# sp-uhh/disentangled-vae

Hardware: AMD Instinct MI355X
Metric: spectrogram frames/sec (train step), M2 VAE 513-bin (higher is better)
Workload: dtype bf16x3; 1 GPU; M2 VAE train step (fwd+ELBO+bwd+Adam), x_dim 513, y_dim 513, z 16, h [128,128], 8192 frames/step/GPU, 16 kHz / 1024-pt STFT power frames; parallelism=dp1, min_hbm_bytes_per_frame=4168

## Files before the change

### disentangled-vae_amd/csrc/rows_common.hpp

```cpp
#pragma once
#include "fused_tiles.hpp"
#include "apply_types.hpp"
#include "../../include/dvae_train.h"

namespace dvae {
namespace fused {

__device__ __forceinline__ void philox_normal4(unsigned long long seed, unsigned long long frame, unsigned long long step, unsigned draw,
                                               float (&out)[4]) {
    unsigned c0 = (unsigned)frame, c1 = (unsigned)(frame >> 32), c2 = (unsigned)step, c3 = ((unsigned)(step >> 32) << 8) | draw;
    unsigned k0 = (unsigned)seed, k1 = (unsigned)(seed >> 32);
#pragma unroll
    for (int r = 0; r < 10; ++r) {
        const unsigned h0 = __umulhi(0xD2511F53u, c0), l0 = 0xD2511F53u * c0;
        const unsigned h1 = __umulhi(0xCD9E8D57u, c2), l1 = 0xCD9E8D57u * c2;
        c0 = h1 ^ c1 ^ k0; c1 = l1; c2 = h0 ^ c3 ^ k1; c3 = l0;
        k0 += 0x9E3779B9u; k1 += 0xBB67AE85u;
    }
    const float u0 = ((float)(c0 >> 8) + 0.5f) * (1.f / 16777216.f), u1 = ((float)(c1 >> 8) + 0.5f) * (1.f / 16777216.f);
    const float u2 = ((float)(c2 >> 8) + 0.5f) * (1.f / 16777216.f), u3 = ((float)(c3 >> 8) + 0.5f) * (1.f / 16777216.f);
    const float ra = sqrtf(-2.f * __logf(u0)), rb = sqrtf(-2.f * __logf(u2));
    float sa, ca, sb, cb;
    __sincosf(6.283185307179586f * u1, &sa, &ca);
    __sincosf(6.283185307179586f * u3, &sb, &cb);
// ... 129 lines not shown
                if (fbase + l31 >= col_limit) f[j] = P::cvt(0.f);
            }
            stash_store16(dbase, (l31 * E + gq * 32 * E) * (int)sizeof(T), f);
        }
    }
}

template <typename P, bool F16 = false, typename RowOf>
__device__ __forceinline__ void load_rows_to_lds(const float* __restrict__ src, int ld, int ncols, int pcols, int64_t b0, int64_t B,
                                                 typename P::T* U, int ldu, int tid, RowOf rowof, float* xf = nullptr,
                                                 float* log2sum = nullptr, float eps = 0.f) {
    const int total = TB * pcols;
    for (int idx = tid; idx < total; idx += 256) {
        const int row = idx / pcols, col = idx - row * pcols;
        float v = 0.f;
        if (col < ncols && b0 + row < B) {
            v = src[rowof(row) * ld + col];
            if (log2sum && col < XD - 1) *log2sum += __builtin_amdgcn_logf(v + eps);
        }
        if constexpr (F16 && P::NP == 2) {
            const float vs = v * X16::XS;
            const typename P::T vh = X16::hi<typename P::T>(vs);
            U[row * ldu + col] = vh;
            U[Pl<P>::lds + row * ldu + col] = X16::hi<typename P::T>(vs - X16::val(vh));
        } else {
            const typename P::T vh = P::cvt(v);
            U[row * ldu + col] = vh;
            if constexpr (P::NP == 2) U[Pl<P>::lds + row * ldu + col] = P::cvt(v - (float)vh);
        }
        if (xf && col < ncols) xf[row * ncols + col] = v;
    }
}

constexpr int NQ513 = 17;
struct __attribute__((packed, aligned(4))) F4U { f32x4 v; };
#ifndef R2_IN_NT
#define R2_IN_NT 0
#endif
typedef f32x4 f32x4_a4 __attribute__((aligned(4)));
__device__ __forceinline__ f32x4 ld_in4(const float* p) {
#if R2_IN_NT >= 1
    return __builtin_nontemporal_load(reinterpret_cast<const f32x4_a4*>(p));
#else
    return reinterpret_cast<const F4U*>(p)->v;
#endif
}
__device__ __forceinline__ f32x4 ld_in4_again(const float* p) {
#if R2_IN_NT >= 2
    return __builtin_nontemporal_load(reinterpret_cast<const f32x4_a4*>(p));
#else
    return reinterpret_cast<const F4U*>(p)->v;
#endif
}
template <int I0, int I1, typename RowOf>
__device__ __forceinline__ void tile513_issue_part(const float* __restrict__ base, RowOf rowof, f32x4 (&v)[NQ513], int tid) {
#pragma unroll
    for (int i = I0; i < I1; ++i) {
        const int c = tid + 256 * i;
        v[i] = ld_in4(base + rowof(c >> 7) * XD + 4 * (c & 127));
    }
}
template <typename RowOf>
__device__ __forceinline__ void tile513_issue_last(const float* __restrict__ base, RowOf rowof, f32x4 (&v)[NQ513], int tid) {
    v[16][0] = base[rowof(tid & 31) * XD + XD - 1];
}
template <typename RowOf>
__device__ __forceinline__ void tile513_issue(const float* __restrict__ base, RowOf rowof, f32x4 (&v)[NQ513], int tid) {
    tile513_issue_part<0, 16>(base, rowof, v, tid);
    tile513_issue_last(base, rowof, v, tid);
    __builtin_amdgcn_sched_barrier(0);
}
template <typename P, int I0, int I1, bool F16 = false>
__device__ __forceinline__ void tile513_commit_part(const f32x4 (&v)[NQ513], typename P::T* U, int ldu, int tid, float* xf, unsigned long long& lo_bits) {
    typedef typename P::Pack4 Pack4;
#pragma unroll
    for (int i = I0; i < I1; ++i) {
        const int c = tid + 256 * i;
        const int row = c >> 7, col = 4 * (c & 127);
        if (xf) {
            float* d = xf + row * XD + col;
            d[0] = v[i][0]; d[1] = v[i][1]; d[2] = v[i][2]; d[3] = v[i][3];
        }
        if constexpr (F16 && P::NP == 2) {
            Pack4 pk, pl;
#pragma unroll
            for (int j = 0; j < 4; ++j) {
                const float vs = v[i][j] * X16::XS;
                pk[j] = X16::hi<typename P::T>(vs);
                pl[j] = X16::hi<typename P::T>(vs - X16::val(pk[j]));
            }
            *reinterpret_cast<Pack4*>(U + row * ldu + col) = pk;
            *reinterpret_cast<Pack4*>(U + Pl<P>::lds + row * ldu + col) = pl;
            continue;
        }
        Pack4 pk;
        pk[0] = P::cvt(v[i][0]); pk[1] = P::cvt(v[i][1]); pk[2] = P::cvt(v[i][2]); pk[3] = P::cvt(v[i][3]);
        *reinterpret_cast<Pack4*>(U + row * ldu + col) = pk;
        if constexpr (P::NP == 2) {
            Pack4 pl;
            pl[0] = P::cvt(v[i][0] - (float)pk[0]); pl[1] = P::cvt(v[i][1] - (float)pk[1]);
            pl[2] = P::cvt(v[i][2] - (float)pk[2]); pl[3] = P::cvt(v[i][3] - (float)pk[3]);
            *reinterpret_cast<Pack4*>(U + Pl<P>::lds + row * ldu + col) = pl;
            lo_bits |= __builtin_bit_cast(unsigned long long, pl) & 0x7fff7fff7fff7fffull;
        }
    }
}
template <typename P, int PCOLS, bool F16 = false>
__device__ __forceinline__ void tile513_commit_last(const f32x4 (&v)[NQ513], typename P::T* U, int ldu, int tid, float* xf, unsigned long long& lo_bits) {
    constexpr int PADC = PCOLS - XD;
    if (tid < TB) {
        if (xf) xf[tid * XD + XD - 1] = v[16][0];
        if constexpr (F16 && P::NP == 2) {
            const float vs = v[16][0] * X16::XS;
            const typename P::T vh = X16::hi<typename P::T>(vs);
            U[tid * ldu + XD - 1] = vh;
            U[Pl<P>::lds + tid * ldu + XD - 1] = X16::hi<typename P::T>(vs - X16::val(vh));
        } else {
        const typename P::T vh = P::cvt(v[16][0]);
        U[tid * ldu + XD - 1] = vh;
        if constexpr (P::NP == 2) {
            const typename P::T vl = P::cvt(v[16][0] - (float)vh);
            U[Pl<P>::lds + tid * ldu + XD - 1] = vl;
            if ((float)vl != 0.f) lo_bits |= 1ull;
        }
        }
    }
    for (int idx = tid; idx < TB * PADC; idx += 256) {
        const int r = idx / PADC, c = XD + idx - r * PADC;
        U[r * ldu + c] = P::cvt(0.f);
        if constexpr (P::NP == 2) U[Pl<P>::lds + r * ldu + c] = P::cvt(0.f);
    }
// ... 98 lines not shown
```

### disentangled-vae_amd/csrc/rows_helper.inc

```
        const int hw = wave_u - ROWS_CHAIN_WAVES, ht = tid - 64 * ROWS_CHAIN_WAVES;
        constexpr bool XFH = P::XF16 && NP == 2;
        constexpr int NBT = Ld<T>::nbias;
        constexpr int NB = (NBT + 255) / 256;
        float bvv[NB];
        auto load_bias = [&]() __attribute__((always_inline)) {
#pragma unroll
            for (int q = 0; q < NB; ++q) {
                int i = ht + 256 * q;
                i = i < NBT ? i : NBT - 1;
                const float* src;
                int k;
                if (i < OB2) { src = g.b1; k = i; }
                else if (i < OBMV) { src = g.b2; k = i - OB2; }
                else if (i < OBMV + ZD) { src = g.bmu; k = i - OBMV; }
                else if (i < OB3) { src = g.blv; k = i - OBMV - ZD; }
                else if (i < OB4) { src = g.b3; k = i - OB3; }
                else if (i < OB5) { src = g.b4; k = i - OB4; }
                else if (i < OB5 + NO) { src = g.b5; k = i - OB5; k = k < XD ? k : XD - 1; }
                else { src = g.w5last; k = i - OB5 - NO; }
                if constexpr (DEFER) bvv[q] = __hip_atomic_load(src + k, __ATOMIC_RELAXED, __HIP_MEMORY_SCOPE_AGENT);
                else bvv[q] = src[k];
            }
        };
        auto store_bias = [&]() __attribute__((always_inline)) {
// ... 5 lines not shown
        };
        if constexpr (!DEFER) load_bias();
        auto fill_rows = [&](int tl_, int half) {
            if (ht < TB) {
                const int64_t bf = (int64_t)tl_ * TB + ht;
                const int64_t br = bf < g.B ? bf : g.B - 1;
                int64_t r = g.rows[br];
                if (r < 0 || r >= g.n_rows) { r = 0; if (g.bad_rows && bf < g.B) atomicAdd(g.bad_rows, 1); }
                rowsrc[half * TB + ht] = r;
            }
        };
        typedef Sched<P, YP, YENC, (OFFL ? P::PDO : P::PD), INFO> SCc;
        typedef HSched<P, YP, YENC, DH, INFO> HS;
        typedef WStream<P, HS, DH> HWS;
        HWS hws;
        if constexpr (HS::any) {
            hws.rs = __builtin_amdgcn_make_buffer_rsrc(const_cast<void*>(g.wcopy), 0, (int)g.wcopy_bytes, 0x00020000);
            hws.voff = lane * 16;
            hws.pl = g.wpl_bytes;
            auto mo = [&](const void* Wp) { return (unsigned)((const char*)Wp - (const char*)g.wcopy); };
            constexpr unsigned FBB = HS::FBB;
            const unsigned tw = (unsigned)hw * FBB;
            hws.sb[H_W1X] = mo(g.W1s) + tw + (unsigned)SCc::NX1 * 4u * FBB;
            hws.sb[H_W3Y] = mo(g.W3s) + tw + (unsigned)(ZD / KS) * 4u * FBB;
            hws.sb[H_W3Z] = mo(g.W3s) + tw;
            hws.sb[H_PAD] = mo(g.W1s);
            if constexpr (INFO) { hws.sb[H_C1] = mo(g.Wc1s) + tw;  hws.sb[H_C2] = mo(g.Wc2s) + tw;  hws.sb[H_C2T] = mo(g.Wc2t) + tw; }
            else { hws.sb[H_C1] = hws.sb[H_C2] = hws.sb[H_C2T] = 0; }
            if constexpr (INFO) hws.fill();
        }
        const T* const Urh = U + l31 * LDU + h * E;
        const T* const Zbrh = Zb + l31 * LDZ + h * E;
        float lsum2 = 0.f;
        f32x4 xv[NQ513], yv[NQ513];
        bool x_in_regs = false;
        bool y_in_regs = false;
        const bool st1 = MODE != 1 && !(g.ablate & 1), st2 = MODE != 1 && !(g.ablate & 2) && (g.stash_inputs & 2), st2x = MODE != 1 && !(g.ablate & 2) && (g.stash_inputs & 1);
        for (int it = 0; it < ntl; ++it) {
            const int tile = tile0 + it * (int)gridDim.x;
            const int64_t b0 = (int64_t)tile * TB;
            const bool full = (b0 + TB) <= g.B;
            const int64_t* const rsrc = rowsrc + (it & 1) * TB;
            auto rowof = [&](int r) -> int64_t {
                if (gather) return rsrc[r];
                const int64_t br = b0 + r;
                return br < g.B ? br : g.B - 1;
            };
            int tl = ht;
            asm volatile("" : "+v"(tl));
            const bool yfast = Y513 && g.fasty && full;
            bool y_early = it > 0 && y_in_regs;
            if (it == 0) {
                if (gather) { fill_rows(tile, 0); wg_barrier(); }
                if (g.fastx && full) {
                    tile513_issue(g.x, rowof, xv, tl);
                    if constexpr (!DEFER) store_bias();
#if R2_EARLY_Y
                    if (YP > 0 && Y513 && g.fasty) {
                        unsigned long long lb = 0ull;
                        static_for<0, 4>([&](auto qc) {
                            constexpr int Q = decltype(qc)::value;
                            tile513_issue_part<4 * Q, 4 * Q + 4>(g.y, rowof, yv, tl);
                            __builtin_amdgcn_sched_barrier(0);
                            tile513_commit_part<P, 4 * Q, 4 * Q + 4, XFH>(xv, U, LDU, tl, nullptr, lb);
                            __builtin_amdgcn_sched_barrier(0);
                        });
                        tile513_issue_last(g.y, rowof, yv, tl);
                        __builtin_amdgcn_sched_barrier(0);
                        tile513_commit_last<P, ROWS_XP, XFH>(xv, U, LDU, tl, nullptr, lb);
                        y_early = true;
                    } else
#endif
                    {
                        tile513_commit<P, ROWS_XP, XFH>(xv, U, LDU, tl);
#pragma unroll
                        for (int i = 0; i < NQ513; ++i) yv[i] = f32x4{0.f, 0.f, 0.f, 0.f};
                    }
                } else {
#pragma unroll
                    for (int i = 0; i < NQ513; ++i) { xv[i] = f32x4{0.f, 0.f, 0.f, 0.f}; yv[i] = f32x4{0.f, 0.f, 0.f, 0.f}; }
                    if constexpr (!DEFER) store_bias();
                    load_rows_to_lds<P, XFH>(g.x, g.ldx, XD, ROWS_XP, b0, g.B, U, LDU, tl, rowof, nullptr, OFFL ? &lsum2 : nullptr, g.elbo_eps);
                }
                if constexpr (INFO) {
                    for (int i = ht; i < 6 * HD + 2; i += 256) {
                        const int q = i / HD, k = i - q * HD;
                        float v;
                        if (q == 0) v = g.bc1[k]; else if (q == 1) v = g.bc2[k]; else if (q == 2) v = g.wc3[k];
                        else if (q == 3) v = g.ba1[k]; else if (q == 4) v = g.ba2[k]; else if (q == 5) v = g.wa3[k];
                        else v = k == 0 ? g.bc3[0] : g.ba3[0];
                        Binfo[i] = v;
                    }
                }
                if (ht == 0) flags[0] = 0;
                if constexpr (DEFER) {
                    wg_barrier();
                    load_bias();
                    store_bias();
                }
                wg_barrier();
                if constexpr (OFFL) { if (g.fastx && full) lsum2 += tile513_log2sum(xv, g.elbo_eps, tl); }
            }
            if constexpr (HS::n(H_W1X) > 0) {
                f32x16 hacc;
                zero_acc<P>(hacc);
                hws.fill();
                gemm_seg<P, HS, DH, H_W1X, HWS, XFH>(hacc, hws, Urh + SCc::NX1 * 2 * E);
#pragma unroll
                for (int r = 0; r < 16; ++r) keep[r * 256 + ht] = XFH ? hacc[r] * X16::ACC : hacc[r];
            }
            float c1r[16], c2r[16], w3c[16];
            float bce_c = 0.f, ylab = 0.f;
            if constexpr (INFO) {
                ylab = g.y[rowof(l31) * g.ldy];
                if (it > 0) hws.fill();
                f32x16 cacc;
                zero_acc<P>(cacc);
                gemm_seg<P, HS, DH, H_C1, HWS, XFH>(cacc, hws, Urh);
                float bvc[16];
                bias16(Binfo + OBC1, 32 * hw, h, bvc);
#pragma unroll
                for (int r = 0; r < 16; ++r) c1r[r] = fmaxf((XFH ? cacc[r] * X16::ACC : cacc[r]) + bvc[r], 0.f);
            }
            f32x16 accy;
            int yplanes = NP;
            int ydirty = 0;
            if constexpr (NP == 2 && YP > 0) { if (g.ylo_skip && st2) ydirty = g.ylo_dirty[tile]; }
            if (YP > 0) {
                if (Y513 && yfast && !y_early) tile513_issue(g.y, rowof, yv, tl);
                R2_HSTAMP(16);
                if (st2x && !XFH) stash_from_lds<P>(U, LDU, ROWS_XP, NO, (T*)g.xT, g.spl, g.Bp, b0, tl);
                R2_HSTAMP(17);
                wg_barrier();
                if constexpr (HS::HELPY && HS::n(H_W1X) == 0) hws.fill();
                R2_HSTAMP(18);
                bool any = false;
                if (Y513 && yfast) tile513_commit<P, ROWS_XP>(yv, U, LDU, tl, nullptr, NP == 2 ? &any : nullptr);
                else load_rows_to_lds<P>(g.y, g.ldy, g.ydim, YP, b0, g.B, U, LDU, tl, rowof);
                R2_HSTAMP(19);
                if constexpr (NP == 2) {
                    if (Y513 && yfast) {
                    } else {
                        constexpr int YPD = YP > 0 ? YP : 1;
                        for (int idx = tl; idx < TB * YP; idx += 256) any |= (float)U[Pl<P>::lds + (idx / YPD) * LDU + idx % YPD] != 0.f;
                    }
                    if (__ballot(any) != 0ull && lane == 0) atomicOr(&flags[0], 1);
                }
                R2_HSTAMP(20);
                if constexpr (INFO) put_lds<P>(c1r, U + IMA, LDU, 32 * hw, l31, h);
                wg_barrier();
                if constexpr (NP == 2) {
                    const bool ylo_t = __builtin_amdgcn_readfirstlane(flags[0]) != 0;
                    if (g.ylo_skip && st2) {
                        ydirty = __builtin_amdgcn_readfirstlane(ydirty);
                        yplanes = (ylo_t || ydirty != 0) ? 2 : 1;
                        if (ht == 0) {
                            if (ylo_t) *g.ylo_epoch = g.launch_id;
                            if ((ylo_t ? 1 : 0) != ydirty) g.ylo_dirty[tile] = ylo_t ? 1 : 0;
                        }
                    }
                }
#if !R2_LATE_Y
                if (st2) stash_from_lds<P>(U, LDU, YP, (YP + 31) / 32 * 32, (T*)g.yT, g.spl, g.Bp, b0, tl, 0, 1 << 30, yplanes);
#endif
                if constexpr (HS::HELPY) {
                    const bool ylo = NP == 2 && __builtin_amdgcn_readfirstlane(flags[0]) != 0;
                    zero_acc<P>(accy);
                    if (!R2_YLOSEG) gemm_seg<P, HS, DH, H_W3Y>(accy, hws, Urh, ylo);
                    else if (ylo) gemm_seg<P, HS, DH, H_W3Y>(accy, hws, Urh, true);
                    else gemm_seg<P, HS, DH, H_W3Y>(accy, hws, Urh, false);
                }
                if constexpr (INFO) {
                    f32x16 a2c;
                    zero_acc<P>(a2c);
                    gemm_seg<P, HS, DH, H_C2>(a2c, hws, Urh + IMA);
                    float bvc[16];
                    bias16(Binfo + OBC2, 32 * hw, h, bvc);
                    bias16(Binfo + OWC3, 32 * hw, h, w3c);
                    float pd = 0.f;
#pragma unroll
                    for (int r = 0; r < 16; ++r) { c2r[r] = fmaxf(a2c[r] + bvc[r], 0.f); pd = fmaf(w3c[r], c2r[r], pd); }
                    put_lds<P>(c2r, U + IMB, LDU, 32 * hw, l31, h);
                    pd += __shfl_xor(pd, 32, 64);
                    if (h == 0) red2[hw * 32 + l31] = pd;
                }
            } else {
                if (st2x && !XFH) stash_from_lds<P>(U, LDU, ROWS_XP, NO, (T*)g.xT, g.spl, g.Bp, b0, tl);
                if constexpr (HS::n(H_W1X) > 0) wg_barrier();
            }
            wg_barrier();
            if constexpr (INFO) {
                const bool live_h = (b0 + l31) < g.B;
                const float logit = red2[l31] + red2[32 + l31] + red2[64 + l31] + red2[96 + l31] + Binfo[OS3];
                const float p = 1.f / (1.f + P::exp_(-logit));
                const float lp = P::log_(p + g.elbo_eps), lq = P::log_(1.f - p + g.elbo_eps);
                bce_c = (live_h && h == 0 && hw == 0) ? -(ylab * lp + (1.f - ylab) * lq) : 0.f;
                const float u = live_h ? -g.invB * (ylab / (p + g.elbo_eps) - (1.f - ylab) / (1.f - p + g.elbo_eps)) : 0.f;
                const float dpre3 = u * p * (1.f - p);
                float dv2[16];
#pragma unroll
                for (int r = 0; r < 16; ++r) dv2[r] = c2r[r] > 0.f ? w3c[r] * dpre3 : 0.f;
                put_lds<P>(dv2, U + IMC, LDU, 32 * hw, l31, h);
                if (st1) {
                    stash_tile<P>(U + IMA, LDU, 32 * hw, (T*)g.c1T + (int64_t)hw * 32 * g.Bp, g.spl, b0, l31, h);
                    stash_tile<P>(U + IMB, LDU, 32 * hw, (T*)g.c2T + (int64_t)hw * 32 * g.Bp, g.spl, b0, l31, h);
                    if (hw == 0 && h == 0) {
                        T* d3 = (T*)g.dc3T + (b0 / KS) * (64 * E) + (l31 / E) * 32 * E + (l31 % E);
                        const T d3h = P::cvt(dpre3 * g.alpha);
                        *d3 = d3h;
                        if constexpr (NP == 2) d3[g.spl] = P::cvt(dpre3 * g.alpha - (float)d3h);
                    }
                }
            }
            if (st1) stash_tile<P>(Ha, LDH, 32 * hw, (T*)g.h1T + (int64_t)hw * 32 * g.Bp, g.spl, b0, l31, h);
#ifndef R2_XSP
#define R2_XSP 1
#endif
            if constexpr (XFH && !INFO && R2_XSP == 0) { if (st2x) xstash_reload<P, 0, 4>(g.x, g.ldx, rowof, b0, g.B, (T*)g.xT, g.spl, g.Bp, tl); }
#if R2_LATE_Y
            if (YP > 0 && st2) stash_from_lds<P>(U, LDU, YP, (YP + 31) / 32 * 32, (T*)g.yT, g.spl, g.Bp, b0, tl, 0, R2_YSPREAD, yplanes);
#endif
            wg_barrier();
            if constexpr (INFO) {
                f32x16 a3c;
                zero_acc<P>(a3c);
                gemm_seg<P, HS, DH, H_C2T>(a3c, hws, Urh + IMC);
                float dv1[16];
#pragma unroll
                for (int r = 0; r < 16; ++r) dv1[r] = c1r[r] > 0.f ? a3c[r] : 0.f;
                put_lds<P>(dv1, U + IMA, LDU, 32 * hw, l31, h);
                if (st1) stash_tile<P>(U + IMC, LDU, 32 * hw, (T*)g.dc2T + (int64_t)hw * 32 * g.Bp, g.spl, b0, l31, h, g.alpha);
            }
            if (st1) stash_tile<P>(Hb, LDH, 32 * hw, (T*)g.h2T + (int64_t)hw * 32 * g.Bp, g.spl, b0, l31, h);
            if constexpr (XFH && !INFO) {
                if (st2x) {
                    if constexpr (R2_XSP == 0) xstash_reload<P, 4, 9>(g.x, g.ldx, rowof, b0, g.B, (T*)g.xT, g.spl, g.Bp, tl);
                    else if constexpr (R2_XSP == 1) xstash_reload<P, 0, 9>(g.x, g.ldx, rowof, b0, g.B, (T*)g.xT, g.spl, g.Bp, tl);
                    else xstash_reload<P, 0, 5>(g.x, g.ldx, rowof, b0, g.B, (T*)g.xT, g.spl, g.Bp, tl);
                }
            }
#if R2_LATE_Y
            if (YP > 0 && st2) stash_from_lds<P>(U, LDU, YP, (YP + 31) / 32 * 32, (T*)g.yT, g.spl, g.Bp, b0, tl, R2_YSPREAD, 1 << 30, yplanes);
#endif
            wg_barrier();
            if constexpr (HS::HELPY) {
                f32x16 az;
                zero_acc<P>(az);
                gemm_seg<P, HS, DH, H_W3Z>(az, hws, Zbrh);
                float hv[16], bv[16];
                bias16(Bias + OB3, 32 * hw, h, bv);
#pragma unroll
                for (int r = 0; r < 16; ++r) hv[r] = P::tanh_(az[r] + accy[r] + bv[r]);
                put_lds<P>(hv, Ha, LDH, 32 * hw, l31, h);
            }
            if (hw == 0 && st1) stash_tile<P>(Zb, LDZ, 0, (T*)g.zT, g.spl, b0, l31, h);
            if constexpr (XFH && !INFO && R2_XSP == 2) { if (st2x) xstash_reload<P, 5, 9>(g.x, g.ldx, rowof, b0, g.B, (T*)g.xT, g.spl, g.Bp, tl); }
            if (ht == 0) flags[0] = 0;
            if constexpr (INFO) {
                if (st1) stash_tile<P>(U + IMA, LDU, 32 * hw, (T*)g.dc1T + (int64_t)hw * 32 * g.Bp, g.spl, b0, l31, h, g.alpha);
                const float sa = g.gamma - g.beta;
                wg_barrier();
                if (st1) stash_tile<P>(Ha, LDH, 32 * hw, (T*)g.a1T + (int64_t)hw * 32 * g.Bp, g.spl, b0, l31, h);
                if constexpr (XFH) { if (st2x) xstash_reload<P, 0, 5>(g.x, g.ldx, rowof, b0, g.B, (T*)g.xT, g.spl, g.Bp, tl); }
                wg_barrier();
                if (st1) {
                    stash_tile<P>(Hb, LDH, 32 * hw, (T*)g.a2T + (int64_t)hw * 32 * g.Bp, g.spl, b0, l31, h);
                    if (hw == 0 && h == 0) {
                        const bool live_h = (b0 + l31) < g.B;
                        const float logit = red2[l31] + red2[32 + l31] + red2[64 + l31] + red2[96 + l31] + Binfo[OS3 + 1];
                        const float p = 1.f / (1.f + P::exp_(-logit));
                        const float u = live_h ? -g.invB * (ylab / (p + g.elbo_eps) - (1.f - ylab) / (1.f - p + g.elbo_eps)) : 0.f;
                        const float dpre3 = u * p * (1.f - p);
                        T* d3 = (T*)g.da3T + (b0 / KS) * (64 * E) + (l31 / E) * 32 * E + (l31 % E);
                        const T d3h = P::cvt(dpre3 * sa);
// ... 137 lines not shown
```

### disentangled-vae_amd/csrc/rows_prologue.inc

```
    typedef typename P::T T;
    typedef typename P::Frag Frag;
    constexpr int E = P::E, KS = P::KSTEP, NP = P::NP;
    constexpr int LDU = Ld<T>::u, LDH = Ld<T>::hh, LDZ = Ld<T>::z;
    constexpr bool Y513 = (YP == ROWS_XP);
#ifndef R2_OFFL
#define R2_OFFL 1
#endif
#ifndef R2_LATE_Y
#define R2_LATE_Y 1
#endif
#ifndef R2_EARLY_Y
#define R2_EARLY_Y 1
#endif
#ifndef R2_DH
#define R2_DH 6
#endif
#ifndef R2_HPRIO
#define R2_HPRIO 0
#endif
#ifndef R2_YSPREAD
#define R2_YSPREAD 8
#endif
#ifndef R2_YLOSEG
#define R2_YLOSEG 0
#endif
#ifndef R2_STAGGER
#define R2_STAGGER 0
#endif
    constexpr bool OFFL = R2_OFFL && MODE == 0 && NP == 2;
    extern __shared__ __attribute__((aligned(16))) char smem[];
    T* const U = reinterpret_cast<T*>(smem);
    T* const Ha = U + TB * LDU;
    T* const Hb = Ha + TB * LDH;
    T* const Zb = Hb + TB * LDH;
    typedef Lds2<P, INFO> LD2;
    float* const Bias = reinterpret_cast<float*>(smem + LD2::o_bias);
    float* const red = reinterpret_cast<float*>(smem + LD2::o_red);
    int* const flags = reinterpret_cast<int*>(smem + LD2::o_flags);
    int64_t* const rowsrc = reinterpret_cast<int64_t*>(smem + LD2::o_rows);
    float* const Binfo = reinterpret_cast<float*>(smem + LD2::o_info);
    float* const red2 = reinterpret_cast<float*>(smem + LD2::o_red2);
    float* const dzs = reinterpret_cast<float*>(smem + LD2::o_dzu);
    constexpr int OBC1 = 0, OBC2 = HD, OWC3 = 2 * HD, OBA1 = 3 * HD, OBA2 = 4 * HD, OWA3 = 5 * HD, OS3 = 6 * HD;
    constexpr int IMA = 32, IMB = 160, IMC = 288;
    float* const keep = reinterpret_cast<float*>(smem + LD2::o_keep);
    float* const keepz = reinterpret_cast<float*>(smem + LD2::o_keepz);
    constexpr int OB1 = 0, OB2 = HD, OBMV = 2 * HD, OB3 = 2 * HD + 32, OB4 = 3 * HD + 32, OB5 = 4 * HD + 32;

    constexpr int DH = R2_DH;
    const int tid = threadIdx.x, lane = tid & 63;
    const int wave_u = __builtin_amdgcn_readfirstlane(tid >> 6);
    const int l31 = lane & 31, h = lane >> 5;
    const bool gather = g.rows != nullptr;
#ifndef R2_XCDMAP
#define R2_XCDMAP 0
#endif
    int tile0 = (int)blockIdx.x;
#if R2_XCDMAP
    if ((gridDim.x & 7) == 0 && (g.ntiles % (int)gridDim.x) == 0) tile0 = (int)(blockIdx.x & 7) * (int)(gridDim.x >> 3) + (int)(blockIdx.x >> 3);
#endif
    const int ntl = (g.ntiles - tile0 + (int)gridDim.x - 1) / (int)gridDim.x;
```

### disentangled-vae_amd/csrc/train_rows2.hip

```cpp
#include <math.h>
#include <stdlib.h>
#include "fused_tiles.hpp"
#include "rows_common.hpp"
#include "wstream.hpp"
#include "apply_common.hpp"
#include "rows_shared.hpp"
#include "../../include/dvae_train.h"

namespace dvae {
namespace fused {

template <typename P, int YP, bool YENC, int MODE, bool INFO = false, bool DEFER = false>
__global__ __launch_bounds__(512) void vae_rows2_kernel(const RowsArgs g) {
    static_assert(!INFO || (MODE == 0 && YP == 16 && !YENC), "M2_info: train step, 1-dim label, encoder on x only");
    static_assert(!DEFER || (MODE == 0 && !INFO && sizeof(typename P::T) == 2), "deferred optimizer step: M1 / M2 train step, bf16 copies");
#define ROWS_XP XP
#define ROWS_PREFETCH 1
#define ROWS_CHAIN_WAVES 4
#include "rows_prologue.inc"
    if (wave_u < 4) {
        const int cw = wave_u, fb = 32 * cw;
        constexpr int D = OFFL ? P::PDO : P::PD;
        typedef Sched<P, YP, YENC, D, INFO> SC;
        typedef HSched<P, YP, YENC, DH, INFO> HS;
#ifndef R2_DEFER_WAUX
#define R2_DEFER_WAUX 0
#endif
        typedef WStream<P, SC, D, DEFER ? R2_DEFER_WAUX : R2_WAUX> WS;
        constexpr unsigned FBB = SC::FBB;
        WS ws;
        ws.rs = __builtin_amdgcn_make_buffer_rsrc(const_cast<void*>(g.wcopy), 0, (int)g.wcopy_bytes, 0x00020000);
        ws.voff = lane * 16;
        ws.pl = g.wpl_bytes;
        {
            auto mo = [&](const void* Wp) { return (unsigned)((const char*)Wp - (const char*)g.wcopy); };
#ifdef R2_SAMEW
            const unsigned tw = 0;
#else
            const unsigned tw = (unsigned)cw * FBB;
#endif
            constexpr unsigned KB1 = (XP / KS) * 4 * FBB, KB3 = (ZD / KS) * 4 * FBB;
            ws.sb[G_W1X] = mo(g.W1s) + tw;  ws.sb[G_W1Y] = mo(g.W1s) + tw + KB1;
            ws.sb[G_W2] = mo(g.W2s) + tw;   ws.sb[G_WMV] = mo(g.Wmvs);
            ws.sb[G_W3Y] = mo(g.W3s) + tw + KB3;  ws.sb[G_W3Z] = mo(g.W3s) + tw;
            ws.sb[G_W4] = mo(g.W4s) + tw;
            ws.sb[G_W5A] = mo(g.W5s) + (unsigned)cw * FBB;        ws.sb[G_W5B] = mo(g.W5s) + (unsigned)(cw + 4) * FBB;
            ws.sb[G_W5C] = mo(g.W5s) + (unsigned)(cw + 8) * FBB;  ws.sb[G_W5D] = mo(g.W5s) + (unsigned)(cw + 12) * FBB;
            ws.sb[G_W5T] = mo(g.W5t) + tw;  ws.sb[G_W4T] = mo(g.W4t) + tw;  ws.sb[G_W3ZT] = mo(g.W3zt);
            ws.sb[G_WMVT] = mo(g.Wmvt) + tw;  ws.sb[G_W2T] = mo(g.W2t) + tw;  ws.sb[G_PAD] = mo(g.W1s);
            if constexpr (INFO) {
                ws.sb[G_A1] = mo(g.Wa1s) + tw;  ws.sb[G_A2] = mo(g.Wa2s) + tw;  ws.sb[G_A2T] = mo(g.Wa2t) + tw;  ws.sb[G_A1T] = mo(g.Wa1t);
            } else { ws.sb[G_A1] = ws.sb[G_A2] = ws.sb[G_A2T] = ws.sb[G_A1T] = 0; }
        }
        if constexpr (DEFER) {
            if (g.defer.have) {
                T* const tile = reinterpret_cast<T*>(keep) + cw * DeferLds<T, NP>::wave_elems;
                if (!(g.defer.diag & 1))
                for (int un = cw * (int)gridDim.x + (int)blockIdx.x; un < 4 * g.defer.ntasks; un += 4 * (int)gridDim.x)
                    defer_unit<T, NP>(g.defer.a, g.defer.tasks[un >> 2], un & 3, tile, lane, g.defer.diag);
                asm volatile("s_waitcnt vmcnt(0)" ::: "memory");
                if (lane == 0)
                    __hip_atomic_fetch_add(g.defer.shard + 32 * (((int)blockIdx.x * 4 + cw) & (DEFER_SHARDS - 1)), 1u, __ATOMIC_RELAXED, __HIP_MEMORY_SCOPE_AGENT);
                if (cw == 0 && !(g.defer.diag & 2)) {
                    const int nw = 4 * (int)gridDim.x, sh = lane & (DEFER_SHARDS - 1);
                    const unsigned want = g.defer.seq_arrive * (unsigned)((nw - sh + DEFER_SHARDS - 1) / DEFER_SHARDS);
                    const unsigned long long deadline = wall_clock64() + g.defer.timeout_ticks;
                    bool ok = true;
                    for (unsigned it_ = 0;; ++it_) {
                        const unsigned have = __hip_atomic_load(g.defer.shard + 32 * sh, __ATOMIC_RELAXED, __HIP_MEMORY_SCOPE_AGENT);
                        if (__ballot((int)(have - want) < 0) == 0ull) break;
                        if ((it_ & 15u) == 0u && wall_clock64() >= deadline) { ok = false; break; }
                        __builtin_amdgcn_s_sleep(1);
                    }
                    if (!ok && lane == 0) __hip_atomic_store(g.defer.err, 1u, __ATOMIC_RELAXED, __HIP_MEMORY_SCOPE_AGENT);
                }
            }
            wg_barrier();
        }
        ws.fill();
        const T* const Ur = U + l31 * LDU + h * E;
        const T* const Har = Ha + l31 * LDH + h * E;
        const T* const Hbr = Hb + l31 * LDH + h * E;
        const T* const Zbr = Zb + l31 * LDZ + h * E;
        const bool w0 = cw == 0;
        constexpr int mode = MODE;
        double tot_rec = 0.0, tot_kl = 0.0, tot_bc = 0.0, tot_ba = 0.0;

        for (int it = 0; it < ntl; ++it) {
            const int tile = tile0 + it * (int)gridDim.x;
            const int64_t b0 = (int64_t)tile * TB;
            const bool live = (b0 + l31) < g.B;
            const int64_t* const rsrc = rowsrc + (it & 1) * TB;
            float rec_lane = 0.f, kl_lane = 0.f;
            R2_STAMP(0);
            if (g.dbg && tid == 0) g.dbg[(size_t)blockIdx.x * 32 + 30] = clock64();
            float ep_r[8];
            if (w0) {
                int64_t br = b0 + l31; br = br < g.B ? br : g.B - 1;
                if (g.eps != nullptr) {
                    const f32x4 e0 = *reinterpret_cast<const f32x4*>(g.eps + br * ZD + 4 * h);
                    const f32x4 e1 = *reinterpret_cast<const f32x4*>(g.eps + br * ZD + 8 + 4 * h);
#pragma unroll
                    for (int jq = 0; jq < 4; ++jq) { ep_r[jq] = live ? e0[jq] : 0.f; ep_r[4 + jq] = live ? e1[jq] : 0.f; }
                } else {
                    frame_noise8(g.rng_seed, (unsigned long long)br, g.rng_step, h, ep_r);
#pragma unroll
                    for (int jq = 0; jq < 8; ++jq) ep_r[jq] = live ? ep_r[jq] : 0.f;
                }
            }
            if (it == 0) {
                if (gather) wg_barrier();
                wg_barrier();
            }
            R2_STAMP(1);
#if R2_STAGGER
            if (it == 0) { for (int q = 0; q < (int)((blockIdx.x >> 3) & 7); ++q) __builtin_amdgcn_s_sleep(R2_STAGGER); }
#endif
            f32x16 acc;
            zero_acc<P>(acc);
            constexpr bool XF = P::XF16 && NP == 2;
            gemm_seg<P, SC, D, G_W1X, WS, XF>(acc, ws, Ur);
            if constexpr (XF) {
#pragma unroll
                for (int r = 0; r < 16; ++r) acc[r] *= X16::ACC;
            }
            R2_STAMP(2);
            bool ylo = false;
            if (YP > 0) {
                wg_barrier();
                wg_barrier();
                ylo = NP == 2 && __builtin_amdgcn_readfirstlane(flags[0]) != 0;
                if (!R2_YLOSEG) gemm_seg<P, SC, D, G_W1Y>(acc, ws, Ur, ylo);
                else if (ylo) gemm_seg<P, SC, D, G_W1Y>(acc, ws, Ur, true);
                else gemm_seg<P, SC, D, G_W1Y>(acc, ws, Ur, false);
            } else if constexpr (HS::n(H_W1X) > 0) wg_barrier();
            if constexpr (HS::n(H_W1X) > 0) {
#pragma unroll
                for (int r = 0; r < 16; ++r) acc[r] += keep[r * 256 + tid];
            }
            float hv[16], bv[16];
            R2_STAMP(3);
            bias16(Bias + OB1, fb, h, bv);
#pragma unroll
            for (int r = 0; r < 16; ++r) { hv[r] = P::tanh_(acc[r] + bv[r]); keep[r * 256 + tid] = hv[r]; }
            put_lds<P>(hv, Ha, LDH, fb, l31, h);
            wg_barrier();
            R2_STAMP(4);
            zero_acc<P>(acc);
            gemm_seg<P, SC, D, G_W2>(acc, ws, Har);
            bias16(Bias + OB2, fb, h, bv);
#pragma unroll
            for (int r = 0; r < 16; ++r) { hv[r] = P::tanh_(acc[r] + bv[r]); keep[(16 + r) * 256 + tid] = hv[r]; }
            put_lds<P>(hv, Hb, LDH, fb, l31, h);
            wg_barrier();
            R2_STAMP(5);
            zero_acc<P>(acc);
            gemm_seg<P, SC, D, G_WMV>(acc, ws, Hbr, true, w0);
            if (w0) {
                float zv[16];
                bias16(Bias + OBMV, 0, h, bv);
#pragma unroll
                for (int r = 0; r < 8; ++r) {
                    const float mu = acc[r] + bv[r], lv = acc[r + 8] + bv[r + 8];
                    keepz[r * 64 + lane] = mu; keepz[(8 + r) * 64 + lane] = lv;
                    zv[r] = fmaf(P::exp_(0.5f * lv), ep_r[r], mu);
                    zv[r + 8] = 0.f;
                    if (live) kl_lane += lv - mu * mu - P::exp_(lv);
                }
                put_lds<P>(zv, Zb, LDZ, 0, l31, h);
                if (mode == 1 && live) {
                    const int64_t o = (b0 + l31) * ZD + 4 * h;
#pragma unroll
                    for (int q = 0; q < 2; ++q) {
                        *reinterpret_cast<f32x4*>(g.out_mu + o + 8 * q) = f32x4{acc[4 * q] + bv[4 * q], acc[4 * q + 1] + bv[4 * q + 1], acc[4 * q + 2] + bv[4 * q + 2], acc[4 * q + 3] + bv[4 * q + 3]};
// ... 243 lines not shown
                    const float kmu = mode == 0 ? mu * g.invB : gu[8 + r];
                    const float klv = mode == 0 ? -0.5f * g.invB * (1.f - P::exp_(lv)) : gu[16 + r];
                    dml[r] = live ? dz + kmu : 0.f;
                    dml[r + 8] = live ? dz * ep_r[r] * (0.5f * P::exp_(0.5f * lv)) + klv : 0.f;
                }
                put_lds<P>(dml, Zb, LDZ, 0, l31, h);
            }
            wg_barrier();
            R2_STAMP(12);
            zero_acc<P>(acc);
            gemm_seg<P, SC, D, G_WMVT>(acc, ws, Zbr);
#pragma unroll
            for (int r = 0; r < 16; ++r) { const float hk = keep[(16 + r) * 256 + tid]; dv[r] = acc[r] * (1.f - hk * hk); }
            put_lds<P>(dv, Hb, LDH, fb, l31, h);
            wg_barrier();
            R2_STAMP(13);
            zero_acc<P>(acc);
            gemm_seg<P, SC, D, G_W2T>(acc, ws, Hbr);
            { f32x16 dummy; zero_acc<P>(dummy); gemm_seg<P, SC, D, G_PAD>(dummy, ws, Hbr, true, false); }
#pragma unroll
            for (int r = 0; r < 16; ++r) { const float hk = keep[r * 256 + tid]; dv[r] = acc[r] * (1.f - hk * hk); }
            put_lds<P>(dv, Ha, LDH, fb, l31, h);
            wg_barrier();
            R2_STAMP(14);
            if (!live) rec_lane = 0.f;
            const float rs = wave_sum(rec_lane), ks = wave_sum(kl_lane);
            if (lane == 0) { red[cw] = rs; red[4 + cw] = ks; }
            if constexpr (INFO) { if (w0) { const float bas = wave_sum(bce_a); if (lane == 0) red2[129] = bas; } }
            wg_barrier();
            if (tid == 0) {
                if constexpr (INFO) { tot_bc += (double)red2[128]; tot_ba += (double)red2[129]; }
                tot_rec += (double)red[0] + (double)red[1] + (double)red[2] + (double)red[3];
                if constexpr (OFFL)
                    tot_rec += (double)red[8] + (double)red[9] + (double)red[10] + (double)red[11]
                             - 0.6931471805599453 * ((double)red[12] + (double)red[13] + (double)red[14] + (double)red[15]);
                tot_kl += -0.5 * (double)red[4];
            }
        }
        R2_STAMP(15);
        if (g.dbg && tid == 0) g.dbg[(size_t)blockIdx.x * 32 + 31] = clock64();
        if (tid == 0) {
            g.partials[4 * blockIdx.x] = tot_rec;
            g.partials[4 * blockIdx.x + 1] = tot_kl;
            g.partials[4 * blockIdx.x + 2] = tot_bc;
            g.partials[4 * blockIdx.x + 3] = tot_ba;
        }
    } else {
#include "rows_helper.inc"
    }
}

#undef ROWS_XP
#undef ROWS_CHAIN_WAVES
template <typename P, int YP, bool YENC, int MODE, bool INFO = false, bool DEFER = false>
static int launch_rows2_m(const RowsArgs& a, int grid, hipStream_t s) {
    const size_t lds = Lds2<P, INFO>::bytes;
    static bool attr_done[64] = {};
    int dev = 0;
    (void)hipGetDevice(&dev);
    if (dev < 0 || dev >= 64) dev = 0;
    if (!attr_done[dev]) {
        hipError_t e = hipFuncSetAttribute((const void*)vae_rows2_kernel<P, YP, YENC, MODE, INFO, DEFER>, hipFuncAttributeMaxDynamicSharedMemorySize, (int)lds);
        if (e != hipSuccess) { set_error("hipFuncSetAttribute(rows2 kernel, %zu B LDS): %s", lds, hipGetErrorString(e)); return (int)e; }
        attr_done[dev] = true;
    }
    hipLaunchKernelGGL((vae_rows2_kernel<P, YP, YENC, MODE, INFO, DEFER>), dim3(grid), dim3(512), lds, s, a);
    DVAE_LAUNCH_OK("vae_rows2_kernel");
    return 0;
}

template <typename P, int YP, bool YENC>
static int launch_rows2_t(const RowsArgs& a, int grid, hipStream_t s) {
    if (a.mode == 1) return launch_rows2_m<P, YP, YENC, 1>(a, grid, s);
    if (a.mode == 2) return launch_rows2_m<P, YP, YENC, 2>(a, grid, s);
#ifdef DVAE_DIAG
    if (a.defer.on) return launch_rows2_m<P, YP, YENC, 0, false, true>(a, grid, s);
#else
    if (a.defer.on) { set_error("rows2 kernel: the deferred optimizer step exists in the diagnostic build only (build.py --diag)"); return DVAE_E_UNSUPPORTED; }
#endif
    return launch_rows2_m<P, YP, YENC, 0>(a, grid, s);
}

int launch_rows2(int precision, int model, int y_dim, const RowsArgs& a, int grid, hipStream_t s) {
    const bool m2 = model == DVAE_MODEL_M2;
    if (model == DVAE_MODEL_M2_INFO) {
        if (a.mode != 0) { set_error("rows2 kernel: M2_info runs the fused train step only (mode %d)", a.mode); return DVAE_E_UNSUPPORTED; }
        if (precision == DVAE_PREC_BF16X3) return launch_rows2_m<PolX3v2, 16, false, 0, true>(a, grid, s);
        if (precision == DVAE_PREC_BF16) return launch_rows2_m<PolBF16v2, 16, false, 0, true>(a, grid, s);
    }
    if (model == DVAE_MODEL_M2_DEC) {
        if (precision == DVAE_PREC_BF16X3) return launch_rows2_t<PolX3v2, 16, false>(a, grid, s);
        if (precision == DVAE_PREC_BF16) return launch_rows2_t<PolBF16v2, 16, false>(a, grid, s);
    }
    if (precision == DVAE_PREC_BF16X3) {
        if (!m2) return launch_rows2_t<PolX3v2, 0, false>(a, grid, s);
        if (y_dim == 1) return launch_rows2_t<PolX3v2, 16, true>(a, grid, s);
        return launch_rows2_t<PolX3v2, 528, true>(a, grid, s);
    }
    if (precision == DVAE_PREC_BF16) {
        if (!m2) return launch_rows2_t<PolBF16v2, 0, false>(a, grid, s);
        if (y_dim == 1) return launch_rows2_t<PolBF16v2, 16, true>(a, grid, s);
        return launch_rows2_t<PolBF16v2, 528, true>(a, grid, s);
    }
    set_error("rows2 kernel: unsupported precision %d", precision);
    return DVAE_E_UNSUPPORTED;
}
// ... 9 lines not shown
```

### disentangled-vae_amd/csrc/wstream.hpp

```cpp
#pragma once
#include <type_traits>
#include "fused_tiles.hpp"

#ifndef R2_WAUX
#define R2_WAUX 0
#endif
#ifndef R2_NX1
#define R2_NX1 33
#endif
#ifndef R2_HELPY
#define R2_HELPY 0
#endif

namespace dvae {
namespace fused {

enum { G_W1X, G_W1Y, G_W2, G_WMV, G_W3Y, G_A1, G_A2, G_A2T, G_A1T, G_W3Z, G_W4, G_W5A, G_W5B, G_W5C, G_W5D, G_W5T, G_W4T, G_W3ZT, G_WMVT, G_W2T, G_PAD, G_N };

template <typename P, int YP, bool YENC, int D, bool INFO = false> struct Sched {
    static constexpr int KS = P::KSTEP;
    static constexpr int NSEG = G_N;
    static constexpr unsigned FBB = 64u * P::E * sizeof(typename P::T);
    static constexpr int NX1 = (R2_NX1 > 0 && R2_NX1 < XP / KS) ? R2_NX1 : XP / KS;
    static constexpr bool HELPY = R2_HELPY && YP == XP;
// ... 24 lines not shown
             : s == H_C1 ? (INFO ? XP / KS : 0) : (s == H_C2 || s == H_C2T) ? (INFO ? HD / KS : 0) : 0;
    }
    static constexpr int sum_raw() { int t = 0; for (int s = 0; s < H_PAD; ++s) t += raw(s); return t; }
    static constexpr int pad = 0;
    static constexpr int total = sum_raw();
    static constexpr bool any = sum_raw() > 0;
    static constexpr bool WRAP = false;
    static constexpr int n(int s) { return s == H_PAD ? pad : raw(s); }
    static constexpr int start(int s) { int t = 0; for (int i = 0; i < s; ++i) t += n(i); return t; }
    static constexpr int seg_of(int q) { int s = 0; while (q >= start(s) + n(s)) ++s; return s; }
    static constexpr unsigned stride(int s) { return 4u * FBB; }
};

template <int I, int N, typename F>
__device__ __forceinline__ void static_for(F&& f) {
    if constexpr (I < N) { f(std::integral_constant<int, I>{}); static_for<I + 1, N>(f); }
}

template <typename P, typename SC, int D, int AUX = R2_WAUX> struct WStream {
    typename P::Frag r[D][P::NP];
    __amdgpu_buffer_rsrc_t rs;
    int voff;
    unsigned pl;
    unsigned sb[SC::NSEG];
    unsigned cur;
    template <int Q> __device__ __forceinline__ void req() {
        constexpr int s = SC::seg_of(Q);
        if constexpr (Q == SC::start(s)) cur = sb[s];
        else cur += SC::stride(s);
        asm volatile("" : "+s"(cur));
        const u32x4 v0 = __builtin_amdgcn_raw_buffer_load_b128(rs, voff, cur, AUX);
        r[Q % D][0] = __builtin_bit_cast(typename P::Frag, v0);
        if constexpr (P::NP == 2) {
            const u32x4 v1 = __builtin_amdgcn_raw_buffer_load_b128(rs, voff, cur + pl, AUX);
            r[Q % D][1] = __builtin_bit_cast(typename P::Frag, v1);
        }
    }
    template <int S, int SLOT> __device__ __forceinline__ void req_next() {
        cur += SC::stride(S);
        asm volatile("" : "+s"(cur));
        const u32x4 v0 = __builtin_amdgcn_raw_buffer_load_b128(rs, voff, cur, AUX);
        r[SLOT][0] = __builtin_bit_cast(typename P::Frag, v0);
        if constexpr (P::NP == 2) {
            const u32x4 v1 = __builtin_amdgcn_raw_buffer_load_b128(rs, voff, cur + pl, AUX);
            r[SLOT][1] = __builtin_bit_cast(typename P::Frag, v1);
        }
    }
    __device__ __forceinline__ void fill() {
        static_for<0, (D < SC::total ? D : SC::total)>([&](auto ic) { this->template req<decltype(ic)::value>(); });
        __builtin_amdgcn_sched_barrier(0);
    }
};

template <typename P, typename SC, int D, int S, typename WS, bool F16 = false>
__device__ __forceinline__ void gemm_seg(f32x16& acc, WS& w, const typename P::T* brow, bool blo = true, bool active = true) {
    typedef typename P::Frag Frag;
    constexpr int N = SC::n(S), Q0 = SC::start(S), STR = 2 * P::E;
    if constexpr (N > 0) {
        constexpr int BD = N < P::BDMAX ? N : P::BDMAX;
        Frag bq[BD][P::NP];
        if (active) {
#pragma unroll
            for (int i = 0; i < BD; ++i) bloadp<P>(bq[i], brow + i * STR);
        }
#ifndef R2_ROLL
#define R2_ROLL 0
#endif
        constexpr int NL = (R2_ROLL && D % BD == 0 && N >= 3 * D) ? (N - D) / D : 0;
        constexpr int NR = NL * D;
        if constexpr (NL > 0) {
            const typename P::T* bl = brow;
#pragma unroll 1
            for (int lap = 0; lap < NL; ++lap) {
                static_for<0, D>([&](auto ic) {
                    constexpr int i = decltype(ic)::value;
                    if (active) {
#ifndef R2_NOMFMA
                        if constexpr (F16) mmap_f16<P>(acc, w.r[(Q0 + i) % D], bq[i % BD]);
                        else mmap<P>(acc, w.r[(Q0 + i) % D], bq[i % BD], blo);
#else
                        acc[0] += (float)w.r[(Q0 + i) % D][0][0] + (float)bq[i % BD][0][0];
#endif
#ifndef R2_NOBLOAD
                        bloadp<P>(bq[i % BD], bl + (i + BD) * STR);
#endif
                    }
#ifndef R2_NOWLOAD
                    w.template req_next<S, (Q0 + i) % D>();
#endif
                    __builtin_amdgcn_sched_barrier(0);
                });
                bl += D * STR;
            }
        }
        static_for<NR, N>([&](auto ic) {
            constexpr int I = decltype(ic)::value;
            if (active) {
#ifndef R2_NOMFMA
                if constexpr (F16) mmap_f16<P>(acc, w.r[(Q0 + I) % D], bq[I % BD]);
                else mmap<P>(acc, w.r[(Q0 + I) % D], bq[I % BD], blo);
#else
                acc[0] += (float)w.r[(Q0 + I) % D][0][0] + (float)bq[I % BD][0][0];
#endif
#ifndef R2_NOBLOAD
                if constexpr (I + BD < N) bloadp<P>(bq[I % BD], brow + (I + BD) * STR);
#endif
            }
#ifndef R2_NOWLOAD
            if constexpr (SC::WRAP) w.template req<(Q0 + I + D) % SC::total>();
            else if constexpr (Q0 + I + D < SC::total) w.template req<Q0 + I + D>();
#endif
            __builtin_amdgcn_sched_barrier(0);
        });
    }
}

}
}
```

Measured before the change: 112.1 million frames/s.

## Overlap first-tile x staging with W1x GEMM via column-grouped commits and barriers

On the first tile, x is loaded with a column-grouped layout (each row split across 8 threads) and committed to LDS in four column groups separated by workgroup barriers. The chain waves' first GEMM segment inserts matching barriers at the group cut points and reloads B fragments there, so it can start on early columns while later columns are still being staged. The offline log2-sum of x is deferred and recomputed from a second load of x later in the tile, moving that work off the opening critical path. This adds extra barriers, a duplicate x read and register pressure from the xr array, and it only affects the first tile of each block.

```diff
diff --git a/disentangled-vae_amd/csrc/rows_common.hpp b/disentangled-vae_amd/csrc/rows_common.hpp
--- a/disentangled-vae_amd/csrc/rows_common.hpp
+++ b/disentangled-vae_amd/csrc/rows_common.hpp
@@ -205,31 +205,49 @@
     return reinterpret_cast<const F4U*>(p)->v;
 #endif
 }
-template <int I0, int I1, typename RowOf>
+template <bool CG>
+__device__ __forceinline__ void tile513_rc(int tid, int i, int& row, int& col) {
+    if constexpr (CG) { row = tid >> 3; col = 32 * i + 4 * (tid & 7); }
+    else { const int c = tid + 256 * i; row = c >> 7; col = 4 * (c & 127); }
+}
+struct XGroups {
+    static constexpr int G = 4;
+    static constexpr int k0(int g) { return g <= 0 ? 0 : g >= G ? XP / 16 : 8 * g + 1; }
+    static constexpr int s1(int g) { return g < 0 ? 0 : g >= G - 1 ? 16 : (k0(g + 1) + 1) / 2; }
+    static constexpr bool cut(int k) { for (int g = 1; g < G; ++g) if (k == k0(g)) return true; return false; }
+    static constexpr int next_cut(int k) { for (int g = 1; g < G; ++g) if (k0(g) > k) return k0(g); return 1 << 30; }
+};
+template <int I0, int I1, bool CG = false, typename RowOf>
 __device__ __forceinline__ void tile513_issue_part(const float* __restrict__ base, RowOf rowof, f32x4 (&v)[NQ513], int tid) {
-#pragma unroll
-    for (int i = I0; i < I1; ++i) {
-        const int c = tid + 256 * i;
-        v[i] = ld_in4(base + rowof(c >> 7) * XD + 4 * (c & 127));
+    if constexpr (CG) {
+        const float* const rp = base + rowof(tid >> 3) * XD + 4 * (tid & 7);
+#pragma unroll
+        for (int i = I0; i < I1; ++i) v[i] = ld_in4(rp + 32 * i);
+    } else {
+#pragma unroll
+        for (int i = I0; i < I1; ++i) {
+            const int c = tid + 256 * i;
+            v[i] = ld_in4(base + rowof(c >> 7) * XD + 4 * (c & 127));
+        }
     }
 }
 template <typename RowOf>
 __device__ __forceinline__ void tile513_issue_last(const float* __restrict__ base, RowOf rowof, f32x4 (&v)[NQ513], int tid) {
     v[16][0] = base[rowof(tid & 31) * XD + XD - 1];
 }
-template <typename RowOf>
+template <bool CG = false, typename RowOf>
 __device__ __forceinline__ void tile513_issue(const float* __restrict__ base, RowOf rowof, f32x4 (&v)[NQ513], int tid) {
-    tile513_issue_part<0, 16>(base, rowof, v, tid);
+    tile513_issue_part<0, 16, CG>(base, rowof, v, tid);
     tile513_issue_last(base, rowof, v, tid);
     __builtin_amdgcn_sched_barrier(0);
 }
-template <typename P, int I0, int I1, bool F16 = false>
+template <typename P, int I0, int I1, bool F16 = false, bool CG = false>
 __device__ __forceinline__ void tile513_commit_part(const f32x4 (&v)[NQ513], typename P::T* U, int ldu, int tid, float* xf, unsigned long long& lo_bits) {
     typedef typename P::Pack4 Pack4;
 #pragma unroll
     for (int i = I0; i < I1; ++i) {
-        const int c = tid + 256 * i;
-        const int row = c >> 7, col = 4 * (c & 127);
+        int row, col;
+        tile513_rc<CG>(tid, i, row, col);
         if (xf) {
             float* d = xf + row * XD + col;
             d[0] = v[i][0]; d[1] = v[i][1]; d[2] = v[i][2]; d[3] = v[i][3];
diff --git a/disentangled-vae_amd/csrc/rows_helper.inc b/disentangled-vae_amd/csrc/rows_helper.inc
--- a/disentangled-vae_amd/csrc/rows_helper.inc
+++ b/disentangled-vae_amd/csrc/rows_helper.inc
@@ -81,7 +81,33 @@
             bool y_early = it > 0 && y_in_regs;
             if (it == 0) {
                 if (gather) { fill_rows(tile, 0); wg_barrier(); }
-                if (g.fastx && full) {
+                if (GRP && g.fastx && full) {
+                    auto opening = [&](auto yc) __attribute__((always_inline)) {
+                        constexpr bool YI = decltype(yc)::value;
+                        constexpr int XG = XGroups::G;
+                        unsigned long long lb = 0ull;
+                        tile513_issue<true>(g.x, rowof, xv, tl);
+                        static_for<0, XG>([&](auto gc) {
+                            constexpr int Gi = decltype(gc)::value;
+                            if constexpr (YI) {
+                                tile513_issue_part<16 * Gi / XG, 16 * (Gi + 1) / XG>(g.y, rowof, yv, tl);
+                                if constexpr (Gi == XG - 1) tile513_issue_last(g.y, rowof, yv, tl);
+                                __builtin_amdgcn_sched_barrier(0);
+                            }
+                            tile513_commit_part<P, XGroups::s1(Gi - 1), XGroups::s1(Gi), XFH, true>(xv, U, LDU, tl, nullptr, lb);
+                            if constexpr (Gi == XG - 1) tile513_commit_last<P, ROWS_XP, XFH>(xv, U, LDU, tl, nullptr, lb);
+                            __builtin_amdgcn_sched_barrier(0);
+                            if constexpr (Gi < XG - 1) wg_barrier();
+                        });
+                        if constexpr (!YI) {
+#pragma unroll
+                            for (int i = 0; i < NQ513; ++i) yv[i] = f32x4{0.f, 0.f, 0.f, 0.f};
+                        }
+                    };
+                    if (R2_EARLY_Y && YP > 0 && Y513 && g.fasty) { opening(std::true_type{}); y_early = true; }
+                    else opening(std::false_type{});
+                    store_bias();
+                } else if (g.fastx && full) {
                     tile513_issue(g.x, rowof, xv, tl);
                     if constexpr (!DEFER) store_bias();
 #if R2_EARLY_Y
@@ -128,8 +154,17 @@
                     store_bias();
                 }
                 wg_barrier();
-                if constexpr (OFFL) { if (g.fastx && full) lsum2 += tile513_log2sum(xv, g.elbo_eps, tl); }
-            }
+                if constexpr (OFFL) { if (!GRP && g.fastx && full) lsum2 += tile513_log2sum(xv, g.elbo_eps, tl); }
+            }
+            const bool relog = GRP && OFFL && it == 0 && g.fastx && full;
+            f32x4 xr[NQ513];
+            auto relog_issue = [&]() __attribute__((always_inline)) {
+                if (relog) tile513_issue(g.x, rowof, xr, tl);
+                else {
+#pragma unroll
+                    for (int i = 0; i < NQ513; ++i) xr[i] = f32x4{0.f, 0.f, 0.f, 0.f};
+                }
+            };
             if constexpr (HS::n(H_W1X) > 0) {
                 f32x16 hacc;
                 zero_acc<P>(hacc);
@@ -177,6 +212,7 @@
                 }
                 R2_HSTAMP(20);
                 if constexpr (INFO) put_lds<P>(c1r, U + IMA, LDU, 32 * hw, l31, h);
+                if constexpr (GRP && OFFL) relog_issue();
                 wg_barrier();
                 if constexpr (NP == 2) {
                     const bool ylo_t = __builtin_amdgcn_readfirstlane(flags[0]) != 0;
@@ -216,7 +252,9 @@
             } else {
                 if (st2x && !XFH) stash_from_lds<P>(U, LDU, ROWS_XP, NO, (T*)g.xT, g.spl, g.Bp, b0, tl);
                 if constexpr (HS::n(H_W1X) > 0) wg_barrier();
-            }
+                if constexpr (GRP && OFFL) relog_issue();
+            }
+            if constexpr (GRP && OFFL && YP > 0) { if (relog) lsum2 += tile513_log2sum(xr, g.elbo_eps, tl); }
             wg_barrier();
             if constexpr (INFO) {
                 const bool live_h = (b0 + l31) < g.B;
@@ -249,6 +287,7 @@
 #if R2_LATE_Y
             if (YP > 0 && st2) stash_from_lds<P>(U, LDU, YP, (YP + 31) / 32 * 32, (T*)g.yT, g.spl, g.Bp, b0, tl, 0, R2_YSPREAD, yplanes);
 #endif
+            if constexpr (GRP && OFFL && YP == 0) { if (relog) lsum2 += tile513_log2sum(xr, g.elbo_eps, tl); }
             wg_barrier();
             if constexpr (INFO) {
                 f32x16 a3c;
diff --git a/disentangled-vae_amd/csrc/rows_prologue.inc b/disentangled-vae_amd/csrc/rows_prologue.inc
--- a/disentangled-vae_amd/csrc/rows_prologue.inc
+++ b/disentangled-vae_amd/csrc/rows_prologue.inc
@@ -28,6 +28,11 @@
 #define R2_STAGGER 0
 #endif
     constexpr bool OFFL = R2_OFFL && MODE == 0 && NP == 2;
+#ifdef ROWS_GROUPED_OPENING
+    constexpr bool GRP = ROWS_GROUPED_OPENING;
+#else
+    constexpr bool GRP = false;
+#endif
     extern __shared__ __attribute__((aligned(16))) char smem[];
     T* const U = reinterpret_cast<T*>(smem);
     T* const Ha = U + TB * LDU;
diff --git a/disentangled-vae_amd/csrc/train_rows2.hip b/disentangled-vae_amd/csrc/train_rows2.hip
--- a/disentangled-vae_amd/csrc/train_rows2.hip
+++ b/disentangled-vae_amd/csrc/train_rows2.hip
@@ -17,6 +17,7 @@
 #define ROWS_XP XP
 #define ROWS_PREFETCH 1
 #define ROWS_CHAIN_WAVES 4
+#define ROWS_GROUPED_OPENING (P::NP == 2 && !DEFER && (R2_NX1 <= 0 || R2_NX1 >= XP / P::KSTEP))
 #include "rows_prologue.inc"
     if (wave_u < 4) {
         const int cw = wave_u, fb = 32 * cw;
@@ -108,6 +109,7 @@
                     for (int jq = 0; jq < 8; ++jq) ep_r[jq] = live ? ep_r[jq] : 0.f;
                 }
             }
+            const bool grp = GRP && it == 0 && g.fastx && (b0 + TB) <= g.B;
             if (it == 0) {
                 if (gather) wg_barrier();
                 wg_barrier();
@@ -119,7 +121,8 @@
             f32x16 acc;
             zero_acc<P>(acc);
             constexpr bool XF = P::XF16 && NP == 2;
-            gemm_seg<P, SC, D, G_W1X, WS, XF>(acc, ws, Ur);
+            if constexpr (GRP) gemm_seg<P, SC, D, G_W1X, WS, XF, XGroups>(acc, ws, Ur, true, true, grp, [] { wg_barrier(); });
+            else gemm_seg<P, SC, D, G_W1X, WS, XF>(acc, ws, Ur);
             if constexpr (XF) {
 #pragma unroll
                 for (int r = 0; r < 16; ++r) acc[r] *= X16::ACC;
@@ -469,6 +472,7 @@
 
 #undef ROWS_XP
 #undef ROWS_CHAIN_WAVES
+#undef ROWS_GROUPED_OPENING
 template <typename P, int YP, bool YENC, int MODE, bool INFO = false, bool DEFER = false>
 static int launch_rows2_m(const RowsArgs& a, int grid, hipStream_t s) {
     const size_t lds = Lds2<P, INFO>::bytes;
diff --git a/disentangled-vae_amd/csrc/wstream.hpp b/disentangled-vae_amd/csrc/wstream.hpp
--- a/disentangled-vae_amd/csrc/wstream.hpp
+++ b/disentangled-vae_amd/csrc/wstream.hpp
@@ -100,8 +100,14 @@
     }
 };
 
-template <typename P, typename SC, int D, int S, typename WS, bool F16 = false>
-__device__ __forceinline__ void gemm_seg(f32x16& acc, WS& w, const typename P::T* brow, bool blo = true, bool active = true) {
+struct NoCuts {
+    static constexpr bool cut(int) { return false; }
+    static constexpr int next_cut(int) { return 1 << 30; }
+};
+struct NoCutFn { __device__ __forceinline__ void operator()() const {} };
+template <typename P, typename SC, int D, int S, typename WS, bool F16 = false, typename CT = NoCuts, typename CutFn = NoCutFn>
+__device__ __forceinline__ void gemm_seg(f32x16& acc, WS& w, const typename P::T* brow, bool blo = true, bool active = true,
+                                         bool cut_now = false, CutFn at_cut = CutFn{}) {
     typedef typename P::Frag Frag;
     constexpr int N = SC::n(S), Q0 = SC::start(S), STR = 2 * P::E;
     if constexpr (N > 0) {
@@ -114,7 +120,7 @@
 #ifndef R2_ROLL
 #define R2_ROLL 0
 #endif
-        constexpr int NL = (R2_ROLL && D % BD == 0 && N >= 3 * D) ? (N - D) / D : 0;
+        constexpr int NL = (R2_ROLL && D % BD == 0 && N >= 3 * D && CT::next_cut(0) > N) ? (N - D) / D : 0;
         constexpr int NR = NL * D;
         if constexpr (NL > 0) {
             const typename P::T* bl = brow;
@@ -143,6 +149,16 @@
         }
         static_for<NR, N>([&](auto ic) {
             constexpr int I = decltype(ic)::value;
+            if constexpr (CT::cut(I)) {
+                if (cut_now) {
+                    at_cut();
+                    if (active) {
+#pragma unroll
+                        for (int i = 0; i < BD; ++i)
+                            if (I + i < N) bloadp<P>(bq[(I + i) % BD], brow + (I + i) * STR);
+                    }
+                }
+            }
             if (active) {
 #ifndef R2_NOMFMA
                 if constexpr (F16) mmap_f16<P>(acc, w.r[(Q0 + I) % D], bq[I % BD]);
@@ -151,7 +167,10 @@
                 acc[0] += (float)w.r[(Q0 + I) % D][0][0] + (float)bq[I % BD][0][0];
 #endif
 #ifndef R2_NOBLOAD
-                if constexpr (I + BD < N) bloadp<P>(bq[I % BD], brow + (I + BD) * STR);
+                if constexpr (I + BD < N) {
+                    if constexpr (CT::next_cut(I) <= I + BD) { if (!cut_now) bloadp<P>(bq[I % BD], brow + (I + BD) * STR); }
+                    else bloadp<P>(bq[I % BD], brow + (I + BD) * STR);
+                }
 #endif
             }
 #ifndef R2_NOWLOAD
```

Result: slower. 109.0 million frames/s (-2.8%).
